# ruanjinchen/Point-Cloud-Flow-Matching

Measured on AMD Instinct MI355X. Metric: train-step points/sec (B=8, N=20000, xyz+rgb) at 1/2/4/8 MI355X; Chamfer ms, higher is better.
Workload: dtype fp32 ContextNet (scatter/gather ops fp32; Conv3d + 1x1 convs as bf16x3 split-operand matrix-core products, fp32 accumulate, ~2^-16 per product vs the reference's default cuDNN TF32 2^-11) + bf16 autocast per-point MLP head (reference AMP config; its per-cloud B-row layers -- embeddings, FiLM affines

## Files before the change

### point-cloud-flow-matching_amd/csrc/pointwise.hip

```cpp
#include <algorithm>
#include <cstdlib>

#include "mfma_x3.hpp"

namespace pcfm {
namespace {

inline int pad_to(int x, int m) { return (x + m - 1) / m * m; }

__device__ __forceinline__ void out_store(float* p, float v) {
#ifndef PCFM_PW_CACHED_STORE
  nt_st(v, p);
#else
  *p = v;
#endif
}
inline int pw_mpad(int m) { return m > 256 ? pad_to(m, 256) : pad_to(m, 128); }

constexpr int kMaxParts = 4;
struct Parts {
  float* p[kMaxParts];
  int off[kMaxParts + 1];
  int n;
  __device__ __forceinline__ float* row(int b, int c, int N) const {
    int i = 0;
#pragma unroll
// ... 117 lines not shown
        const int dm = (e & 3) + 8 * (e >> 2) + 4 * h;
        const int m = mg + dm;
        const int p = p0 + wc * (TN / 2) + j * 32 + r;
        if (m < M && p < N) out_store(yr + (size_t)dm * N + p, acc[i][j][e] + bv[e]);
      }
  }
}

template <int MASK>
__device__ __forceinline__ float swz_xor(float v) {
  return __builtin_bit_cast(
      float, __builtin_amdgcn_ds_swizzle(__builtin_bit_cast(int, v), (MASK << 10) | 0x1f));
}
template <int K, int MASK>
__device__ __forceinline__ void xpose_reduce_stage(float* v, bool upper) {
#pragma unroll
  for (int k = 0; k < K / 2; ++k) {
    const float keep = upper ? v[k + K / 2] : v[k];
    const float send = upper ? v[k] : v[k + K / 2];
    v[k] = keep + swz_xor<MASK>(send);
  }
}

__device__ __forceinline__ void pw256_epilogue(const f32x16 (&acc)[2][2], const Parts& y,
                                               const float* __restrict__ sbias, int b, int nb,
                                               int M, int N, int m0, int p0, int wr, int wc,
                                               int r, int h, float2* __restrict__ stats) {
  const int pw0 = p0 + wc * 64;
#pragma unroll
  for (int i = 0; i < 2; ++i) {
    const int mg = m0 + wr * 64 + i * 32;
    float* __restrict__ yr = y.row(b, min(mg, M - 1), N);
    float bv[16];
#pragma unroll
    for (int e = 0; e < 16; ++e) bv[e] = sbias[mg - m0 + (e & 3) + 8 * (e >> 2) + 4 * h];
#pragma unroll
    for (int j = 0; j < 2; ++j)
#pragma unroll
      for (int e = 0; e < 16; ++e) {
        const int dm = (e & 3) + 8 * (e >> 2) + 4 * h;
        const int m = mg + dm;
        const int p = pw0 + j * 32 + r;
#ifdef PCFM_EXP_PW_NOSTORE
        if (acc[i][j][e] == 1.2345f)
#endif
        if (m < M && p < N) out_store(yr + (size_t)dm * N + p, acc[i][j][e] + bv[e]);
// ... 12 lines not shown
            float, __builtin_amdgcn_readlane(__builtin_bit_cast(int, v0), 32));
        const float sh = h ? s1 : s0;
        sr = r == e ? sh : sr;
        const float d0 = ok0 ? v0 - sh : 0.0f, d1 = ok1 ? v1 - sh : 0.0f;
        v[e] = d0 + d1;
        v[16 + e] = __builtin_fmaf(d1, d1, d0 * d0);
      }
      xpose_reduce_stage<32, 16>(v, r & 16);
      xpose_reduce_stage<16, 8>(v, r & 8);
      xpose_reduce_stage<8, 4>(v, r & 4);
      xpose_reduce_stage<4, 2>(v, r & 2);
      xpose_reduce_stage<2, 1>(v, r & 1);
      const float q = swz_xor<16>(v[0]);
      const int m = mg + (r & 3) + 8 * ((r >> 2) & 3) + 4 * h;
      if (r < 16 && m < M) {
        const float a = v[0], mu_s = a / (float)nv;
        stats[(size_t)m * P + b * ngroups + pw0 / 64] =
            make_float2(sr + mu_s, fmaxf(__builtin_fmaf(-a, mu_s, q), 0.0f));
      }
    }
  }
}

__global__ void __launch_bounds__(512) __attribute__((amdgpu_waves_per_eu(4, 4)))
    pw_gemm256_kernel(const Parts x, const uint16_t* __restrict__ wh,
                      const uint16_t* __restrict__ wl, const float* __restrict__ bias,
                      int bias_bstride, const Parts y, int K, int M, int N, int Kpad,
                      float2* __restrict__ stats = nullptr) {
  constexpr int TM = 256, TN = 128;
  constexpr int A_ELEMS = TM * kLDR, B_ELEMS = TN * kLDR;
  __shared__ __attribute__((aligned(16))) uint16_t lds[2 * A_ELEMS + 2 * B_ELEMS];
  __shared__ float sbias[TM];
  const int b = blockIdx.z, m0 = blockIdx.y * TM, p0 = blockIdx.x * TN;
  const int t = threadIdx.x, lane = t & 63;
  if (t < TM) sbias[t] = bias != nullptr ? bias[b * bias_bstride + min(m0 + t, M - 1)] : 0.0f;
  const int w = __builtin_amdgcn_readfirstlane(t >> 6);
  const int wr = w >> 1, wc = w & 1, r = lane & 31, h = lane >> 5;
  constexpr int CPT = kKT * TN / 512;
  const int sp = t % TN, ch = __builtin_amdgcn_readfirstlane((t / TN) * CPT);
  const int pt = p0 + sp;
  const bool pok = pt < N;
  const int ptc = pok ? pt : N - 1;
  const int arow = t >> 1, ahalf = (t & 1) * 16;
  const int nsteps = Kpad / kKT;

  uint4 ra0 = {}, ra1 = {}, ra2 = {}, ra3 = {};
  float rb[CPT];
  const __amdgpu_buffer_rsrc_t rwh = __builtin_amdgcn_make_buffer_rsrc(
      const_cast<uint16_t*>(wh), (short)0, 0x7FFFFFF0, 0x00020000);
  const __amdgpu_buffer_rsrc_t rwl = __builtin_amdgcn_make_buffer_rsrc(
      const_cast<uint16_t*>(wl), (short)0, 0x7FFFFFF0, 0x00020000);
  const int aoff = ((m0 + arow) * Kpad + ahalf) * 2;
  auto load_a = [&](int s) {
#ifdef PCFM_EXP_PW_NOW
    if (s > 0) return;
#endif
    const int so = s * kKT * 2;
    ra0 = __builtin_bit_cast(uint4, __builtin_amdgcn_raw_buffer_load_b128(rwh, aoff, so, 0));
// ... 70 lines not shown
        }
    }
  };

  load_a(0);
  load_b(0, rb);
  store(0, rb);
  __syncthreads();
  for (int s = 0; s < nsteps; ++s) {
    if (s + 1 < nsteps) {
      load_a(s + 1);
      load_b(s + 1, rb);
    }
    __builtin_amdgcn_sched_barrier(0);
#ifndef PCFM_EXP_PW_NOMFMA
    mfma_step();
#else
    acc[0][0][0] += (float)lds[t];
#endif
    __syncthreads();
    if (s + 1 < nsteps) store(s + 1, rb);
    __syncthreads();
  }
  pw256_epilogue(acc, y, sbias, b, (int)gridDim.z,
                 M, N, m0, p0, wr, wc, r, h, stats);
}

constexpr int kSW = 8;
#ifndef PCFM_PW_STREAM_PF
#define PCFM_PW_STREAM_PF 1
#endif
__device__ __forceinline__ bf16x8 split8(const float (&v)[8], bf16x8& lo) {
  bf16x8 hi;
#pragma unroll
  for (int j = 0; j < 8; ++j) {
    hi[j] = (__bf16)v[j];
    lo[j] = (__bf16)(v[j] - (float)hi[j]);
  }
  return hi;
}

__device__ __forceinline__ const float* uniform_ptr(const float* p) {
  const unsigned long long u = (unsigned long long)p;
  const unsigned lo = __builtin_amdgcn_readfirstlane((unsigned)u);
  const unsigned hi = __builtin_amdgcn_readfirstlane((unsigned)(u >> 32));
  return (const float*)(((unsigned long long)hi << 32) | lo);
}

// ... 463 lines not shown
__global__ void __launch_bounds__(256)
    pw_wgrad_reduce_kernel(const float* __restrict__ part, size_t total, int S,
                           float* __restrict__ dw) {
  __shared__ float red[4][64];
  const int cl = threadIdx.x & 63, grp = threadIdx.x >> 6;
  const size_t i = (size_t)blockIdx.x * 64 + cl;
  float sum = 0.0f;
  if (i < total) {
    int q = grp;
    for (; q + 12 < S; q += 16) {
      float v[4];
#pragma unroll
      for (int u = 0; u < 4; ++u) v[u] = part[(size_t)(q + 4 * u) * total + i];
#pragma unroll
      for (int u = 0; u < 4; ++u) sum = sum + v[u];
    }
    for (; q < S; q += 4) sum = sum + part[(size_t)q * total + i];
  }
  red[grp][cl] = sum;
  __syncthreads();
  if (grp == 0 && i < total) dw[i] = ((red[0][cl] + red[1][cl]) + red[2][cl]) + red[3][cl];
}

bool pw_wgrad_wide(int cin, int cout) {
#ifdef PCFM_PW_NO256
  return false;
#else
  return cin % 256 == 0 && cout % 256 == 0;
#endif
}

int pw_wgrad_splits(int B, int cin, int cout, int N) {
  if (pw_wgrad_wide(cin, cout)) {
    const long long tiles = (long long)(cout / 256) * ((cin + 255) / 256);
    const long long steps = (long long)B * ((N + kKT - 1) / kKT);
    long long s = std::max(1LL, ((long long)kCUs + tiles - 1) / tiles);
    s = std::min(s, std::max(1LL, steps / 16));
    return (int)std::min(s, 256LL);
  }
#ifndef PCFM_PW_WG_BPC
#define PCFM_PW_WG_BPC 2
#endif
#ifndef PCFM_PW_WG_MINSTEPS
#define PCFM_PW_WG_MINSTEPS 8
#endif
#ifndef PCFM_PW_WG_CAP
// ... 38 lines not shown

enum class PwPath { Stream128, Tile256, Tile128, Tile64 };

static PwPath pw_path(int b, int cin, int cout, int n) {
  const int Mpad = pw_mpad(cout), Kpad = pad_to(cin, kKT);
  const long long big = (long long)ceil_div(n, 128) * (Mpad / 128) * b;
#ifndef PCFM_PW_NOSTREAM
  if (Mpad == 128 && Kpad <= 256 && cin % 32 == 0 && cout % 32 == 0) return PwPath::Stream128;
#endif
#ifndef PCFM_PW_NO256
  if (Mpad % 256 == 0 && big / 2 >= 2 * kCUs) return PwPath::Tile256;
#endif
  return big >= 2 * kCUs ? PwPath::Tile128 : PwPath::Tile64;
}

static bool pw_path_has_stats(PwPath p) {
  if (p == PwPath::Stream128) {
    const char* e = std::getenv("PCFM_PW_STREAM_STATS");
    return PCFM_PW_STREAM_PF < 2 && (e == nullptr || e[0] != '0');
  }
  return p == PwPath::Tile256;
}
static int pw_stats_group(PwPath p) { return p == PwPath::Stream128 ? 32 : 64; }

static int pw_gemm_launch(const Parts& x, const void* wsplit, const float* bias, int bias_bstride,
                          int b, int cin, int cout, int n, const Parts& y, hipStream_t st,
                          float2* stats = nullptr) {
  const int Mpad = pw_mpad(cout), Kpad = pad_to(cin, kKT);
  const size_t total = (size_t)Mpad * Kpad;
  const uint16_t* wh = (const uint16_t*)wsplit;
  const PwPath path = pw_path(b, cin, cout, n);
  PCFM_CHECK_ARG(stats == nullptr || pw_path_has_stats(path),
                 "pointwise_gemm: BatchNorm statistics requested for a shape whose kernel has "
                 "no statistics epilogue (b=%d cin=%d cout=%d n=%d)", b, cin, cout, n);
  if (path == PwPath::Stream128) {
    const uint16_t* wl_img = wh + total;
    const long long tiles = (long long)b * ceil_div(n, 32);
    const size_t lds = (size_t)2 * 128 * (Kpad + 8) * sizeof(uint16_t);
    const int per_cu = lds <= 80 * 1024 ? 2 : 1;
    const int slices = Mpad / 128;
    const long long cap = std::max(8LL, ((long long)kCUs * per_cu / slices) & ~7LL);
    const int grid = (int)std::max(1LL, std::min((tiles + kSW - 1) / kSW, cap));
    const void* kfn = nullptr;
    switch (Kpad / 32) {
#define PW_STREAM_CASE(NC)                                                                 \
  case NC:                                                                                 \
    kfn = stats != nullptr ? (const void*)pw_stream128_kernel<NC, true>                    \
                           : (const void*)pw_stream128_kernel<NC, false>;                  \
    break;
      PW_STREAM_CASE(1) PW_STREAM_CASE(2) PW_STREAM_CASE(3) PW_STREAM_CASE(4)
      PW_STREAM_CASE(5) PW_STREAM_CASE(6) PW_STREAM_CASE(7) PW_STREAM_CASE(8)
#undef PW_STREAM_CASE
    }
    const int e = allow_big_lds(kfn);
    if (e) return e;
    void* args[] = {(void*)&x,    (void*)&wh,  (void*)&wl_img, (void*)&bias,
                    (void*)&bias_bstride, (void*)&y, (void*)&cin, (void*)&cout,
                    (void*)&n,    (void*)&b,   (void*)&stats};
    const hipError_t le = hipLaunchKernel(kfn, dim3(grid, slices), dim3(kSW * 64), args, lds, st);
    if (le != hipSuccess) {
      set_error("pointwise_gemm: launch failed");
      return (int)le;
    }
    return check_launch("pointwise_gemm");
  }
  if (path == PwPath::Tile256) {
    const dim3 g256(ceil_div(n, 128), Mpad / 256, b);
    hipLaunchKernelGGL(pw_gemm256_kernel, g256, dim3(512), 0, st, x, wh, wh + total, bias,
                       bias_bstride, y, cin, cout, n, Kpad, stats);
    return check_launch("pointwise_gemm");
  }
  if (path == PwPath::Tile128) {
    hipLaunchKernelGGL((pw_gemm_kernel<128, 128>), dim3(ceil_div(n, 128), Mpad / 128, b),
                       dim3(256), 0, st, x, wh, wh + total, bias, bias_bstride, y, cin, cout, n,
                       Kpad);
  } else {
    hipLaunchKernelGGL((pw_gemm_kernel<64, 64>), dim3(ceil_div(n, 64), Mpad / 64, b), dim3(256),
                       0, st, x, wh, wh + total, bias, bias_bstride, y, cin, cout, n, Kpad);
  }
  return check_launch("pointwise_gemm");
}

static bool make_parts(int np, float* const* ptr, const int* width, int align, Parts& q,
                       int& total) {
  if (np < 1 || np > kMaxParts || ptr == nullptr || width == nullptr) return false;
  q = Parts{};
  q.n = np;
  total = 0;
  for (int i = 0; i < np; ++i) {
    if (width[i] <= 0 || ptr[i] == nullptr) return false;
// ... 11 lines not shown
                                   int cin, int cout, int n, float* y, void* stream) {
  PCFM_CHECK_ARG(pw_ok(b, cin, cout, n), "pointwise_gemm: bad shape b=%d cin=%d cout=%d n=%d", b,
                 cin, cout, n);
  if (b == 0 || n == 0) return PCFM_OK;
  return pw_gemm_launch(one_part(x, cin), wsplit, bias, 0, b, cin, cout, n, one_part(y, cout),
                        (hipStream_t)stream);
}

extern "C" int pcfm_pointwise_bnstats_groups(int b, int cin, int cout, int n) {
  if (!pw_ok(b, cin, cout, n) || b <= 0 || n <= 0) return 0;
  const PwPath p = pw_path(b, cin, cout, n);
  if (!pw_path_has_stats(p)) return 0;
  return b * ceil_div(n, pw_stats_group(p));
}

extern "C" int pcfm_pointwise_gemm_bnstats(const float* x, const void* wsplit, const float* bias,
                                           int b, int cin, int cout, int n, float* y,
                                           float* stats, void* stream) {
  PCFM_CHECK_ARG(pcfm_pointwise_bnstats_groups(b, cin, cout, n) > 0 && stats != nullptr,
                 "pointwise_gemm_bnstats: unsupported shape b=%d cin=%d cout=%d n=%d", b, cin,
                 cout, n);
  return pw_gemm_launch(one_part(x, cin), wsplit, bias, 0, b, cin, cout, n, one_part(y, cout),
                        (hipStream_t)stream, reinterpret_cast<float2*>(stats));
}

extern "C" int pcfm_pointwise_gemm_parts(int nx, const float* const* x, const int* xw,
                                         const void* wsplit, const float* bias, int bias_per_batch,
                                         int b, int n, int ny, float* const* y, const int* yw,
                                         void* stream) {
  Parts px, py;
  int cin = 0, cout = 0;
  PCFM_CHECK_ARG(make_parts(nx, const_cast<float* const*>(x), xw, kKT, px, cin),
                 "pointwise_gemm_parts: bad input parts (1..%d, widths %% %d)", kMaxParts, kKT);
  PCFM_CHECK_ARG(make_parts(ny, y, yw, 128, py, cout),
                 "pointwise_gemm_parts: bad output parts (1..%d, widths %% 128)", kMaxParts);
  PCFM_CHECK_ARG(pw_ok(b, cin, cout, n), "pointwise_gemm_parts: bad shape b=%d cin=%d cout=%d n=%d",
                 b, cin, cout, n);
  if (b == 0 || n == 0) return PCFM_OK;
  return pw_gemm_launch(px, wsplit, bias, bias_per_batch ? cout : 0, b, cin, cout, n, py,
                        (hipStream_t)stream);
}

static int pw_wgrad_launch(const Parts& x, const float* grad_y, int b, int cin, int cout, int n,
                           float* grad_w, void* ws, hipStream_t st) {
  const size_t total = (size_t)cout * cin;
  const int S = pw_wgrad_splits(b, cin, cout, n);
// ... 53 lines not shown
```

### point-cloud-flow-matching_amd/modules/norm_act.py

```python
import torch
import torch.nn.functional as F

__all__ = ["bn_act", "conv_bn_act", "gn_film_residual", "post_gn_film_residual"]

_DEBUG_CHECKS = __import__("os").environ.get("PCFM_DEBUG_CHECKS") == "1"
_BN_FROM_GEMM = __import__("os").environ.get("PCFM_BN_FROM_GEMM", "1") != "0"


class _BNAct(torch.autograd.Function):
    @staticmethod
    def forward(ctx, x, weight, bias, running_mean, running_var, nbt, eps, momentum, slope):
        from pcfm import ops
        y, mean, invstd = ops.bn_act_forward(x, weight, bias, eps, slope, momentum, running_mean,
                                             running_var, nbt)
        ctx.save_for_backward(x, weight, bias, mean, invstd)
        ctx.slope = slope
        return y

    @staticmethod
    def backward(ctx, dy):
        from pcfm import ops
        x, weight, bias, mean, invstd = ctx.saved_tensors
        dx, dgamma, dbeta, _ = ops.bn_act_backward(dy, x, weight, bias, mean, invstd, ctx.slope)
        return dx, dgamma, dbeta, None, None, None, None, None, None


def _fusable(x: torch.Tensor, bn) -> bool:
    if not (x.is_cuda and x.dtype == torch.float32 and x.dim() >= 3 and bn.training
            and bn.affine and bn.track_running_stats and bn.momentum is not None
# ... 8 lines not shown
    if _fusable(x, bn):
        return _BNAct.apply(x.contiguous(), bn.weight, bn.bias, bn.running_mean, bn.running_var,
                            _nbt(bn), float(bn.eps), float(bn.momentum), float(slope))
    y = bn(x)
    return F.relu(y, inplace=True) if slope == 0 else F.leaky_relu(y, slope, inplace=True)


class _PwBnAct(torch.autograd.Function):

    @staticmethod
    def forward(ctx, x, w, b, gamma, beta, rmean, rvar, nbt, eps, momentum, slope):
        from pcfm import ops
        ys = ops.pointwise_forward_bnstats(x, w, b) if _BN_FROM_GEMM else None
        if ys is not None:
            y, stats = ys
            z, mean, invstd = ops.bn_act_forward_parts(y, stats, gamma, beta, eps, slope,
                                                       momentum, rmean, rvar, nbt)
        else:
            y = ops.pointwise_forward(x, w, b)
            z, mean, invstd = ops.bn_act_forward(y, gamma, beta, eps, slope, momentum, rmean,
                                                 rvar, nbt)
        ctx.save_for_backward(x, w, y, gamma, beta, mean, invstd)
        ctx.slope, ctx.has_bias = slope, b is not None
        return z

    @staticmethod
    def backward(ctx, dz):
        from pcfm import ops
        x, w, y, gamma, beta, mean, invstd = ctx.saved_tensors
        dy, dgamma, dbeta, db = ops.bn_act_backward(dz, y, gamma, beta, mean, invstd, ctx.slope,
                                                    want_dbias_in=ctx.has_bias)
        dx = ops.pointwise_backward_data(dy, w) if ctx.needs_input_grad[0] else None
        dw = ops.pointwise_backward_weight(x, dy).view_as(w) if ctx.needs_input_grad[1] else None
        return dx, dw, db, dgamma, dbeta, None, None, None, None, None, None


class _Conv3dBnAct(torch.autograd.Function):

    @staticmethod
    def forward(ctx, x, w, b, gamma, beta, rmean, rvar, nbt, eps, momentum, slope):
        from pcfm import ops
        bsz, cin, r = x.shape[0], x.shape[1], x.shape[2]
        cout = w.shape[0]
        xs = ops.conv3d_split(x)
        y = ops.conv3d_igemm_split(xs, ops.conv3d_prep_weight(w, False), b, bsz, cin, cout, r,
                                   "conv3d_fwd")
        z, mean, invstd = ops.bn_act_forward(y, gamma, beta, eps, slope, momentum, rmean, rvar,
                                             nbt)
        ctx.save_for_backward(xs, w, y, gamma, beta, mean, invstd)
        ctx.slope, ctx.has_bias, ctx.dims = slope, b is not None, (bsz, cin, cout, r)
        return z

    @staticmethod
    def backward(ctx, dz):
        from pcfm import ops
# ... 192 lines not shown
    return x + (y * (1.0 + gamma[:, :, None]) + beta[:, :, None])


_POST_GN_FUSED = __import__("os").environ.get("PCFM_POST_GN_FUSED", "1") != "0"


class _PostGNFiLMRes(torch.autograd.Function):

    @staticmethod
    def forward(ctx, x, w, b, g_bn, bt_bn, rm, rv, nbt, eps, momentum, slope, gn_w, gn_b, gamma,
                beta, groups, gn_eps):
        from pcfm import ops
        ys = ops.pointwise_forward_bnstats(x, w, b) if _BN_FROM_GEMM else None
        if ys is not None:
            y, stats = ys
            mean, invstd = ops.bn_forward_stats(y, eps, momentum, rm, rv, nbt, parts=stats)
        else:
            y = ops.pointwise_forward(x, w, b)
            mean, invstd = ops.bn_forward_stats(y, eps, momentum, rm, rv, nbt)
        out, gm, grs = ops.gn_film_res_forward_bnin(y, mean, invstd, g_bn, bt_bn, slope, gn_w,
                                                    gn_b, gamma, beta, groups, gn_eps)
        ctx.save_for_backward(x, w, y, g_bn, bt_bn, mean, invstd, gn_w, gn_b, gamma, gm, grs)
        ctx.slope, ctx.groups, ctx.has_bias = slope, groups, b is not None
        return out

    @staticmethod
    def backward(ctx, dout):
        from pcfm import ops
        x, w, y, g_bn, bt_bn, mean, invstd, gn_w, gn_b, gamma, gm, grs = ctx.saved_tensors
        dz, dgnw, dgnb, dgamma, dbeta, bnpart = ops.gn_film_res_backward_bnin(
            dout, y, mean, invstd, g_bn, bt_bn, ctx.slope, gn_w, gn_b, gamma, gm, grs, ctx.groups)
        dy, dg_bn, db_bn, db = ops.bn_act_backward_parts(dz, y, g_bn, bt_bn, mean, invstd, bnpart,
                                                         ctx.slope, want_dbias_in=ctx.has_bias)
        del dz
        dx = ops.pointwise_backward_data(dy, w) if ctx.needs_input_grad[0] else None
        dw = ops.pointwise_backward_weight(x, dy).view_as(w) if ctx.needs_input_grad[1] else None
        return (dx, dw, db, dg_bn, db_bn, None, None, None, None, None, None, dgnw, dgnb, dgamma,
                dbeta, None, None)


def post_gn_film_residual(post, norm, x: torch.Tensor, gamma: torch.Tensor, beta: torch.Tensor):
    layers = post.layers
    conv, bn = layers[0], layers[1]
    fused = (_POST_GN_FUSED and len(layers) == 3 and isinstance(layers[2], torch.nn.ReLU)
             and x.is_cuda and x.dtype == torch.float32 and x.dim() == 3
             and _fusable_pre(bn) and hasattr(conv, "x3_ok") and conv.x3_ok(x)
             and conv.bias is not None and isinstance(norm, torch.nn.GroupNorm) and norm.affine
             and x.shape[2] % 4 == 0 and conv.out_channels <= 1024
             and x.shape[0] * conv.out_channels < 65536 and x.shape[0] * x.shape[2] > 1
             and conv.out_channels % norm.num_groups == 0
             and gamma.dtype == torch.float32 and beta.dtype == torch.float32)
    if not fused:
        return gn_film_residual(post(x), norm, gamma, beta)
    return _PostGNFiLMRes.apply(
        x.contiguous(), conv.weight, conv.bias, bn.weight, bn.bias, bn.running_mean,
        bn.running_var, _nbt(bn), float(bn.eps), float(bn.momentum), 0.0, norm.weight, norm.bias,
        gamma, beta, int(norm.num_groups), float(norm.eps))
```

### point-cloud-flow-matching_amd/modules/pvconv.py

```python
import torch
import torch.nn as nn
import torch.nn.functional as TF

import modules.functional as F
from modules.norm_act import (_BN_FROM_GEMM, _fusable_pre, _nbt, _pair_head, _pair_tail,
                              conv_bn_act_pair, pair_fusable)
from modules.se import SE3d
from modules.shared_mlp import SharedMLP
from modules.voxel_conv import VoxelConv3d
from modules.voxelization import Voxelization

__all__ = ["PVConv"]


def _conv_bn_lrelu(cin, cout, kernel_size):
    return [
        VoxelConv3d(cin, cout, kernel_size, stride=1, padding=kernel_size // 2),
        nn.BatchNorm3d(cout, eps=1e-4),
        nn.LeakyReLU(0.1, True),
    ]


_SE_FUSED = __import__("os").environ.get("PCFM_SE_FUSED", "1") != "0"


def _se_scale(m, w1, w2):
    return torch.sigmoid(TF.linear(TF.relu(TF.linear(m, w1)), w2))


# ... 63 lines not shown
        else:
            y_pf, parts = ops.pointwise_forward(f, pw, pb), None
        pm, pis = ops.bn_forward_stats(y_pf, peps, pmom, prm, prv, pnbt, parts=parts)
        xs, y1, m1, is1, z1s, y2 = _pair_head(x, w1, b1, g1, bt1, rm1, rv1, nbt1, w2, b2, eps1,
                                              mom1, slope1, occ)
        mse, m2, is2 = ops.bn_act_forward_rowmean(y2, g2, bt2, eps2, slope2, mom2, rm2, rv2,
                                                  nbt2)
        sw1, sw2 = sw1.contiguous(), sw2.contiguous()
        s, hid = ops.se_mlp_forward(mse, sw1, sw2)
        shared = plans.devox_corners(coords, r)
        out, inds, wgts = ops.trilinear_devoxelize_bn_scale_add(
            r, shared is None, coords, y2, m2, is2, g2, bt2, slope2, s, y_pf,
            add_bn=(pm, pis, pg, pbt, 0.0))
        if shared is not None:
            inds, wgts = shared
        else:
            plans.put_devox_corners(coords, r, inds, wgts)
        ctx.save_for_backward(xs, w1, y1, g1, bt1, m1, is1, z1s, w2, y2, g2, bt2, m2, is2,
                              inds, wgts, mse, s, hid, sw1, sw2, f, pw, y_pf, pg, pbt, pm, pis)
        ctx.points, ctx.r, ctx.occ = coords, r, occ
        ctx.slopes = (slope1, slope2)
        ctx.has_bias = (b1 is not None, b2 is not None, pb is not None)
        ctx.dims = (x.shape[0], x.shape[1], w1.shape[0], w2.shape[0], x.shape[2])
        return out

    @staticmethod
    def backward(ctx, dout):
        from pcfm import ops, plans
        (xs, w1, y1, g1, bt1, m1, is1, z1s, w2, y2, g2, bt2, m2, is2, inds, wgts, mse, s, hid,
         sw1, sw2, f, pw, y_pf, pg, pbt, pm, pis) = ctx.saved_tensors
        dout = dout.contiguous()
        dy_pf, dpg, dpbt, dpb = ops.bn_act_backward(dout, y_pf, pg, pbt, pm, pis, 0.0,
                                                    want_dbias_in=ctx.has_bias[2])
        df = ops.pointwise_backward_data(dy_pf, pw) if ctx.needs_input_grad[18] else None
        dpw = ops.pointwise_backward_weight(f, dy_pf).view_as(pw)
        del dy_pf
        if plans.ENABLED:
            plan = plans.devox_bwd_plan(ctx.points, inds, wgts, ctx.r)
            g = ops.trilinear_devoxelize_backward_planned(dout, plan)
        else:
            g = ops.trilinear_devoxelize_backward(dout, inds, wgts, ctx.r)
        g = g.view(y2.shape)
        rowstats = ops.bn_se_backward_stats(g, y2, m2, is2, g2, bt2, ctx.slopes[1])
        v = y2[0, 0].numel()
        dmv, dsw1, dsw2 = ops.se_mlp_backward(mse, hid, s, rowstats[0], sw1, sw2, 1.0 / v)
        gys2, dg2, dbt2, db2 = ops.bn_se_backward_apply_split(
            g, y2, m2, is2, g2, bt2, s, dmv, rowstats, ctx.slopes[1],
            want_dbias_in=ctx.has_bias[1])
        del g
        dx, dw1, db1, dg1, dbt1, dw2 = _pair_tail(gys2, xs, w1, y1, g1, bt1, m1, is1, z1s, w2,
                                                  ctx.slopes[0], ctx.has_bias[0], ctx.dims,
                                                  ctx.occ, ctx.needs_input_grad[0])
        return (dx, dw1, db1, dg1, dbt1, None, None, None, dw2, db2, dg2, dbt2, None, None, None,
                dsw1, dsw2, None, df, dpw, dpb, dpg, dpbt, None, None, None, None, None, None,
                None, None, None, None, None, None, None)

# ... 94 lines not shown
```

### point-cloud-flow-matching_amd/pcfm/_lib.py

```python
from __future__ import annotations

import ctypes
import os
import threading

_HERE = os.path.dirname(os.path.abspath(__file__))
LIB_PATH = os.path.join(os.path.dirname(_HERE), "csrc", "libpcfm_hip.so")
LIB_PATH = os.environ.get("PCFM_LIB", LIB_PATH)

_P = ctypes.c_void_p
_I = ctypes.c_int
_F = ctypes.c_float
_Z = ctypes.c_size_t
_L = ctypes.c_longlong
_D = ctypes.c_double
_DP = ctypes.POINTER(ctypes.c_double)

SIGNATURES = {
    "pcfm_abi_version": (_I, []),
    "pcfm_last_error": (ctypes.c_char_p, []),
    "pcfm_avg_voxelize_fwd_workspace_bytes": (_Z, [_I, _I, _I, _I]),
    "pcfm_avg_voxelize_fwd": (_I, [_P, _P, _I, _I, _I, _I, _P, _P, _P, _P, _Z, _P]),
    "pcfm_avg_voxelize_bwd": (_I, [_P, _P, _P, _I, _I, _I, _I, _P, _P]),
    "pcfm_trilinear_devoxelize_fwd": (_I, [_P, _P, _I, _I, _I, _I, _I, _P, _P, _P, _P]),
# ... 119 lines not shown
}

ABI_VERSION = 20

ND_SIGNATURES = {
    "pcfm_chamfer_nd_abi_version": (_I, []),
    "pcfm_chamfer_nd_supported": (_I, [_I]),
    "pcfm_chamfer_nd_workspace_bytes": (_Z, [_I, _I, _I, _I]),
    "pcfm_chamfer_nd_fwd": (_I, [_P, _P, _I, _I, _I, _I, _P, _P, _P, _P, _P, _Z, _P]),
    "pcfm_chamfer_nd_bwd": (_I, [_P, _P, _I, _I, _I, _I, _P, _P, _P, _P, _P, _P, _P]),
}

ND_ABI_VERSION = 1

CROSS_SIGNATURES = {
    "pcfm_chamfer_cross_abi_version": (_I, []),
    "pcfm_chamfer_cross_supported": (_I, [_I]),
    "pcfm_chamfer_cross_workspace_bytes": (_Z, [_I, _I, _I, _I, _I]),
    "pcfm_chamfer_cross_fwd": (_I, [_P, _P, _I, _I, _I, _I, _I, _P, _P, _P, _Z, _P]),
}

CROSS_ABI_VERSION = 1

_lock = threading.Lock()
_lib = None


class PcfmError(RuntimeError):
    """A pcfm_* entry point returned a non-zero status."""


def load() -> ctypes.CDLL:
    global _lib
    if _lib is not None:
        return _lib
    with _lock:
        if _lib is None:
            if not os.path.exists(LIB_PATH):
                raise RuntimeError(
                    f"pcfm: HIP library {LIB_PATH} is not built; run "
                    "`python -c 'import __graft_entry__ as g; g.build()'` "
                    "(HIP tensors have no fallback)")
            lib = ctypes.CDLL(LIB_PATH)
            for table in (SIGNATURES, ND_SIGNATURES, CROSS_SIGNATURES):
                for name, (res, args) in table.items():
                    fn = getattr(lib, name)
                    fn.restype = res
                    fn.argtypes = args
            v = lib.pcfm_abi_version()
            if v != ABI_VERSION:
                raise RuntimeError(f"pcfm: ABI version {v} != expected {ABI_VERSION}; rebuild")
            v = lib.pcfm_chamfer_nd_abi_version()
            if v != ND_ABI_VERSION:
                raise RuntimeError(f"pcfm: chamfer_nd ABI version {v} != expected "
                                   f"{ND_ABI_VERSION}; rebuild")
            v = lib.pcfm_chamfer_cross_abi_version()
            if v != CROSS_ABI_VERSION:
                raise RuntimeError(f"pcfm: chamfer_cross ABI version {v} != expected "
                                   f"{CROSS_ABI_VERSION}; rebuild")
            _lib = lib
    return _lib


def call(name: str, *args) -> None:
    lib = load()
    rc = getattr(lib, name)(*args)
    if rc != 0:
        msg = lib.pcfm_last_error().decode(errors="replace")
        raise PcfmError(f"{name} failed (status {rc}): {msg}")


def query(name: str, *args) -> int:
    return int(getattr(load(), name)(*args))
```

### point-cloud-flow-matching_amd/pcfm/ops.py

```python
from __future__ import annotations

import ctypes
import types

import torch

from . import _lib, cpu_ops


def _check_cuda(x: torch.Tensor, name: str) -> None:
    if not (isinstance(x, torch.Tensor) and x.is_cuda):
        raise RuntimeError(f"{name} must be a CUDA tensor")


def _check_contig(x: torch.Tensor, name: str) -> None:
    if not x.is_contiguous():
        raise RuntimeError(f"{name} must be a contiguous tensor")


def _check_float(x: torch.Tensor, name: str) -> None:
    if x.dtype != torch.float32:
        raise RuntimeError(f"{name} must be a float tensor")


# ... 864 lines not shown
        return None
    img = pointwise_prep_weight(weight, False)
    y = torch.empty((b, cout, n), dtype=torch.float32, device=x.device)
    stats = torch.empty((cout, groups, 2), dtype=torch.float32, device=x.device)
    bias_c = bias.contiguous() if bias is not None else None
    bias_p = _ptr(bias_c) if bias_c is not None else None
    with _timed("pointwise_fwd", 2 * b * n * cin * cout, x, "mfma"):
        _lib.call("pcfm_pointwise_gemm_bnstats", _ptr(x), _ptr(img), bias_p, b, cin, cout, n,
                  _ptr(y), _ptr(stats), _stream(x))
    return y, stats


def pointwise_backward_data(grad_y: torch.Tensor, weight: torch.Tensor) -> torch.Tensor:
    _check(grad_y, "grad_output", "f")
    g = grad_y.contiguous()
    b, cout, n = g.shape
    cin = weight.shape[1]
    img = pointwise_prep_weight(weight, True)
    dx = torch.empty((b, cin, n), dtype=torch.float32, device=g.device)
    with _timed("pointwise_bwd_data", 2 * b * n * cin * cout, g, "mfma"):
        _lib.call("pcfm_pointwise_gemm", _ptr(g), _ptr(img), None, b, cout, cin, n, _ptr(dx),
                  _stream(g))
    return dx


def pointwise_backward_weight(x: torch.Tensor, grad_y: torch.Tensor) -> torch.Tensor:
    _check(x, "input", "f")
    _check(grad_y, "grad_output", "f")
    x, g = x.contiguous(), grad_y.contiguous()
    b, cin, n = x.shape
    cout = g.shape[1]
    ws = _workspace(_lib.query("pcfm_pointwise_wgrad_workspace_bytes", b, cin, cout, n), x)
    dw = torch.empty((cout, cin), dtype=torch.float32, device=x.device)
    with _timed("pointwise_wgrad", 2 * b * n * cin * cout, x, "mfma"):
        _lib.call("pcfm_pointwise_wgrad", _ptr(x), _ptr(g), b, cin, cout, n, _ptr(dw), _ptr(ws),
                  ws.numel(), _stream(x))
    return dw


def _parts(ts):
    ptrs = (ctypes.c_void_p * len(ts))(*[_ptr(t) for t in ts])
    widths = (ctypes.c_int * len(ts))(*[int(t.shape[1]) for t in ts])
    return ptrs, widths


def pointwise_forward_parts(xs, weight: torch.Tensor, bias, bias_per_batch: bool = False):
# ... 558 lines not shown
```

Measured before the change: 5.809 million.

## Fuse BatchNorm-backward channel sums into pointwise backward-data GEMM epilogue

Adds a variant of the 256-wide pointwise GEMM whose epilogue, when computing dx for a layer fed by a BN+LeakyReLU, reloads the pre-activation z and produces per-channel partial sums of the masked gradient and gradient*xhat. A small fold kernel reduces these partials, and a handover cache passes them to the upstream BN backward so it can skip its own reduction pass over dy and z. This replaces a full-tensor reduction read with extra epilogue work and z reads inside the GEMM, plus Python-side identity-cache bookkeeping. It only applies on the Tile256 path for supported shapes.

```diff
diff --git a/include/pcfm_bn_parts.h b/include/pcfm_bn_parts.h
--- /dev/null
+++ b/include/pcfm_bn_parts.h
@@ -0,0 +1,27 @@
+#ifndef PCFM_BN_PARTS_H
+#define PCFM_BN_PARTS_H
+
+#include <stddef.h>
+
+#ifdef __cplusplus
+extern "C" {
+#endif
+
+#define PCFM_BN_PARTS_ABI_VERSION 1
+
+int pcfm_bn_parts_abi_version(void);
+
+int pcfm_pointwise_bnbwd_groups(int b, int cin, int cout, int n);
+
+int pcfm_pointwise_gemm_bnbwd(const float* x, const void* wsplit, int b, int cin, int cout, int n,
+                              float* y, const float* z, const float* mean, const float* invstd,
+                              const float* gamma, const float* beta, float slope, float* part,
+                              void* stream);
+
+int pcfm_bn_parts_fold(const float* part, int c, int P, float* folded, void* stream);
+
+#ifdef __cplusplus
+}
+#endif
+
+#endif
diff --git a/point-cloud-flow-matching_amd/csrc/pointwise.hip b/point-cloud-flow-matching_amd/csrc/pointwise.hip
--- a/point-cloud-flow-matching_amd/csrc/pointwise.hip
+++ b/point-cloud-flow-matching_amd/csrc/pointwise.hip
@@ -2,6 +2,7 @@
 #include <cstdlib>
 
 #include "mfma_x3.hpp"
+#include "../../include/pcfm_bn_parts.h"
 
 namespace pcfm {
 namespace {
@@ -165,6 +166,33 @@
   }
 }
 
+struct BnBwdEpi {
+  const float* z;
+  const float* mean;
+  const float* invstd;
+  const float* gamma;
+  const float* beta;
+  float slope;
+  float2* part;
+};
+
+__device__ __forceinline__ void bnbwd_stage(const BnBwdEpi& bw, int m0, int M, int rows, int t,
+                                            float4* __restrict__ sc) {
+  if (t < rows) {
+    const int m = min(m0 + t, M - 1);
+    sc[t] = make_float4(bw.mean[m], bw.invstd[m], bw.gamma[m], bw.beta[m]);
+  }
+}
+
+__device__ __forceinline__ void bnbwd_term(float dz, float z, const float4 c, float slope, bool ok,
+                                           float& sg, float& sgx) {
+  const float xh = (z - c.x) * c.y;
+  float g = __builtin_fmaf(xh, c.z, c.w) > 0.0f ? dz : dz * slope;
+  g = ok ? g : 0.0f;
+  sg += g;
+  sgx += g * xh;
+}
+
 __device__ __forceinline__ void pw256_epilogue(const f32x16 (&acc)[2][2], const Parts& y,
                                                const float* __restrict__ sbias, int b, int nb,
                                                int M, int N, int m0, int p0, int wr, int wc,
@@ -223,18 +251,87 @@
   }
 }
 
-__global__ void __launch_bounds__(512) __attribute__((amdgpu_waves_per_eu(4, 4)))
-    pw_gemm256_kernel(const Parts x, const uint16_t* __restrict__ wh,
-                      const uint16_t* __restrict__ wl, const float* __restrict__ bias,
-                      int bias_bstride, const Parts y, int K, int M, int N, int Kpad,
-                      float2* __restrict__ stats = nullptr) {
+__device__ __forceinline__ void pw256_epilogue_bnbwd(const f32x16 (&acc)[2][2], const Parts& y,
+                                                     int b, int nb, int M, int N, int m0, int p0,
+                                                     int wr, int wc, int r, int h,
+                                                     const BnBwdEpi& bw,
+                                                     const float4* __restrict__ sbn) {
+  const int pw0 = p0 + wc * 64;
+  const int mw = m0 + wr * 64;
+  const bool on0 = pw0 < N && mw < M, on1 = pw0 < N && mw + 32 < M;
+  auto zload = [&](int i, float (&zv)[32]) {
+    const __amdgpu_buffer_rsrc_t rs = __builtin_amdgcn_make_buffer_rsrc(
+        const_cast<float*>(bw.z + ((size_t)b * M + mw + 32 * i) * N), (short)0, 0x7FFFFFF0,
+        0x00020000);
+#pragma unroll
+    for (int j = 0; j < 2; ++j) {
+      const int voff = (4 * h * N + min(pw0 + j * 32 + r, N - 1)) * 4;
+#pragma unroll
+      for (int e = 0; e < 16; ++e)
+        zv[16 * j + e] = __builtin_bit_cast(
+            float,
+            __builtin_amdgcn_raw_buffer_load_b32(rs, voff, ((e & 3) + 8 * (e >> 2)) * N * 4, 0));
+    }
+  };
+  auto sums = [&](int i, const float (&zv)[32]) {
+    const int mg = mw + 32 * i;
+    const int ngroups = (N + 63) / 64, P = nb * ngroups;
+    const bool ok0 = pw0 + r < N, ok1 = pw0 + 32 + r < N;
+    float v[16];
+#pragma unroll
+    for (int e = 0; e < 16; ++e) {
+      const float4 c = sbn[mg - m0 + (e & 3) + 8 * (e >> 2) + 4 * h];
+      float sg = 0.0f, sgx = 0.0f;
+      bnbwd_term(acc[i][0][e] + 0.0f, zv[e], c, bw.slope, ok0, sg, sgx);
+      bnbwd_term(acc[i][1][e] + 0.0f, zv[16 + e], c, bw.slope, ok1, sg, sgx);
+      v[e] = ((r & 16) ? sgx : sg) + swz_xor<16>((r & 16) ? sg : sgx);
+    }
+    xpose_reduce_stage<16, 8>(v, r & 8);
+    xpose_reduce_stage<8, 4>(v, r & 4);
+    xpose_reduce_stage<4, 2>(v, r & 2);
+    xpose_reduce_stage<2, 1>(v, r & 1);
+    const float q = swz_xor<16>(v[0]);
+    const int m = mg + (r & 3) + 8 * ((r >> 2) & 3) + 4 * h;
+    if (r < 16 && m < M) bw.part[(size_t)m * P + b * ngroups + pw0 / 64] = make_float2(v[0], q);
+  };
+  auto stores = [&](int i) {
+    const int mg = mw + 32 * i;
+    float* __restrict__ yr = y.row(b, min(mg, M - 1), N);
+#pragma unroll
+    for (int j = 0; j < 2; ++j)
+#pragma unroll
+      for (int e = 0; e < 16; ++e) {
+        const int dm = (e & 3) + 8 * (e >> 2) + 4 * h;
+        const int p = pw0 + j * 32 + r;
+        if (mg + dm < M && p < N) out_store(yr + (size_t)dm * N + p, acc[i][j][e] + 0.0f);
+      }
+  };
+  float za[32], zb[32];
+  if (on0) {
+    zload(0, za);
+    sums(0, za);
+  }
+  if (on1) zload(1, zb);
+  stores(0);
+  if (on1) sums(1, zb);
+  stores(1);
+}
+
+template <bool BW>
+__device__ __forceinline__ void pw_gemm256_body(const Parts& x, const uint16_t* __restrict__ wh,
+                                                const uint16_t* __restrict__ wl,
+                                                const float* __restrict__ bias, int bias_bstride,
+                                                const Parts& y, int K, int M, int N, int Kpad,
+                                                float2* __restrict__ stats, const BnBwdEpi& bw) {
   constexpr int TM = 256, TN = 128;
   constexpr int A_ELEMS = TM * kLDR, B_ELEMS = TN * kLDR;
   __shared__ __attribute__((aligned(16))) uint16_t lds[2 * A_ELEMS + 2 * B_ELEMS];
   __shared__ float sbias[TM];
+  __shared__ float4 sbn[BW ? TM : 1];
   const int b = blockIdx.z, m0 = blockIdx.y * TM, p0 = blockIdx.x * TN;
   const int t = threadIdx.x, lane = t & 63;
   if (t < TM) sbias[t] = bias != nullptr ? bias[b * bias_bstride + min(m0 + t, M - 1)] : 0.0f;
+  if (BW) bnbwd_stage(bw, m0, M, TM, t, sbn);
   const int w = __builtin_amdgcn_readfirstlane(t >> 6);
   const int wr = w >> 1, wc = w & 1, r = lane & 31, h = lane >> 5;
   constexpr int CPT = kKT * TN / 512;
@@ -351,8 +448,28 @@
     if (s + 1 < nsteps) store(s + 1, rb);
     __syncthreads();
   }
-  pw256_epilogue(acc, y, sbias, b, (int)gridDim.z,
-                 M, N, m0, p0, wr, wc, r, h, stats);
+  if (BW) {
+    pw256_epilogue_bnbwd(acc, y, b, (int)gridDim.z, M, N, m0, p0, wr, wc, r, h, bw, sbn);
+  } else {
+    pw256_epilogue(acc, y, sbias, b, (int)gridDim.z,
+                   M, N, m0, p0, wr, wc, r, h, stats);
+  }
+}
+
+__global__ void __launch_bounds__(512) __attribute__((amdgpu_waves_per_eu(4, 4)))
+    pw_gemm256_kernel(const Parts x, const uint16_t* __restrict__ wh,
+                      const uint16_t* __restrict__ wl, const float* __restrict__ bias,
+                      int bias_bstride, const Parts y, int K, int M, int N, int Kpad,
+                      float2* __restrict__ stats = nullptr) {
+  pw_gemm256_body<false>(x, wh, wl, bias, bias_bstride, y, K, M, N, Kpad, stats, BnBwdEpi{});
+}
+
+__global__ void __launch_bounds__(512) __attribute__((amdgpu_waves_per_eu(4, 4)))
+    pw_gemm256_bnbwd_kernel(const Parts x, const uint16_t* __restrict__ wh,
+                            const uint16_t* __restrict__ wl, const float* __restrict__ bias,
+                            int bias_bstride, const Parts y, int K, int M, int N, int Kpad,
+                            const BnBwdEpi bw) {
+  pw_gemm256_body<true>(x, wh, wl, bias, bias_bstride, y, K, M, N, Kpad, nullptr, bw);
 }
 
 constexpr int kSW = 8;
@@ -862,6 +979,42 @@
   if (grp == 0 && i < total) dw[i] = ((red[0][cl] + red[1][cl]) + red[2][cl]) + red[3][cl];
 }
 
+__global__ void __launch_bounds__(256)
+    bn_parts_fold_kernel(const float2* __restrict__ part, int P, float2* __restrict__ folded) {
+  __shared__ float sh[8];
+  const int c = blockIdx.x, t = threadIdx.x;
+  const float2* __restrict__ pc = part + (size_t)c * P;
+  float a = 0.0f, q = 0.0f;
+  int p = t;
+  for (; p + 3 * 256 < P; p += 4 * 256) {
+    float2 v[4];
+#pragma unroll
+    for (int u = 0; u < 4; ++u) v[u] = pc[p + u * 256];
+#pragma unroll
+    for (int u = 0; u < 4; ++u) {
+      a += v[u].x;
+      q += v[u].y;
+    }
+  }
+  for (; p < P; p += 256) {
+    const float2 v = pc[p];
+    a += v.x;
+    q += v.y;
+  }
+#pragma unroll
+  for (int off = 32; off > 0; off >>= 1) {
+    a += __shfl_xor(a, off, 64);
+    q += __shfl_xor(q, off, 64);
+  }
+  if ((t & 63) == 0) {
+    sh[2 * (t >> 6)] = a;
+    sh[2 * (t >> 6) + 1] = q;
+  }
+  __syncthreads();
+  if (t == 0)
+    folded[c] = make_float2(((sh[0] + sh[2]) + sh[4]) + sh[6], ((sh[1] + sh[3]) + sh[5]) + sh[7]);
+}
+
 bool pw_wgrad_wide(int cin, int cout) {
 #ifdef PCFM_PW_NO256
   return false;
@@ -946,10 +1099,14 @@
   return p == PwPath::Tile256;
 }
 static int pw_stats_group(PwPath p) { return p == PwPath::Stream128 ? 32 : 64; }
+static bool pw_path_has_bnbwd(PwPath p, int cout, int n) {
+  if (cout % 32 != 0 || (long long)n * 128 >= (1LL << 31)) return false;
+  return p == PwPath::Tile256;
+}
 
 static int pw_gemm_launch(const Parts& x, const void* wsplit, const float* bias, int bias_bstride,
                           int b, int cin, int cout, int n, const Parts& y, hipStream_t st,
-                          float2* stats = nullptr) {
+                          float2* stats = nullptr, const BnBwdEpi* bnbwd = nullptr) {
   const int Mpad = pw_mpad(cout), Kpad = pad_to(cin, kKT);
   const size_t total = (size_t)Mpad * Kpad;
   const uint16_t* wh = (const uint16_t*)wsplit;
@@ -957,6 +1114,10 @@
   PCFM_CHECK_ARG(stats == nullptr || pw_path_has_stats(path),
                  "pointwise_gemm: BatchNorm statistics requested for a shape whose kernel has "
                  "no statistics epilogue (b=%d cin=%d cout=%d n=%d)", b, cin, cout, n);
+  PCFM_CHECK_ARG(bnbwd == nullptr ||
+                     (stats == nullptr && bias == nullptr && pw_path_has_bnbwd(path, cout, n)),
+                 "pointwise_gemm: BatchNorm backward sums requested for a shape whose kernel "
+                 "has no such epilogue (b=%d cin=%d cout=%d n=%d)", b, cin, cout, n);
   if (path == PwPath::Stream128) {
     const uint16_t* wl_img = wh + total;
     const long long tiles = (long long)b * ceil_div(n, 32);
@@ -990,6 +1151,11 @@
   }
   if (path == PwPath::Tile256) {
     const dim3 g256(ceil_div(n, 128), Mpad / 256, b);
+    if (bnbwd != nullptr) {
+      hipLaunchKernelGGL(pw_gemm256_bnbwd_kernel, g256, dim3(512), 0, st, x, wh, wh + total, bias,
+                         bias_bstride, y, cin, cout, n, Kpad, *bnbwd);
+      return check_launch("pointwise_gemm");
+    }
     hipLaunchKernelGGL(pw_gemm256_kernel, g256, dim3(512), 0, st, x, wh, wh + total, bias,
                        bias_bstride, y, cin, cout, n, Kpad, stats);
     return check_launch("pointwise_gemm");
@@ -1047,6 +1213,39 @@
                  cout, n);
   return pw_gemm_launch(one_part(x, cin), wsplit, bias, 0, b, cin, cout, n, one_part(y, cout),
                         (hipStream_t)stream, reinterpret_cast<float2*>(stats));
+}
+
+extern "C" int pcfm_bn_parts_abi_version(void) { return PCFM_BN_PARTS_ABI_VERSION; }
+
+extern "C" int pcfm_pointwise_bnbwd_groups(int b, int cin, int cout, int n) {
+  if (!pw_ok(b, cin, cout, n) || b <= 0 || n <= 0) return 0;
+  const PwPath p = pw_path(b, cin, cout, n);
+  if (!pw_path_has_bnbwd(p, cout, n)) return 0;
+  return b * ceil_div(n, pw_stats_group(p));
+}
+
+extern "C" int pcfm_pointwise_gemm_bnbwd(const float* x, const void* wsplit, int b, int cin,
+                                         int cout, int n, float* y, const float* z,
+                                         const float* mean, const float* invstd,
+                                         const float* gamma, const float* beta, float slope,
+                                         float* part, void* stream) {
+  PCFM_CHECK_ARG(pcfm_pointwise_bnbwd_groups(b, cin, cout, n) > 0,
+                 "pointwise_gemm_bnbwd: unsupported shape b=%d cin=%d cout=%d n=%d", b, cin, cout,
+                 n);
+  PCFM_CHECK_ARG(z != nullptr && mean != nullptr && invstd != nullptr && gamma != nullptr &&
+                     beta != nullptr && part != nullptr,
+                 "pointwise_gemm_bnbwd: BatchNorm operands missing");
+  const BnBwdEpi bw{z, mean, invstd, gamma, beta, slope, reinterpret_cast<float2*>(part)};
+  return pw_gemm_launch(one_part(x, cin), wsplit, nullptr, 0, b, cin, cout, n, one_part(y, cout),
+                        (hipStream_t)stream, nullptr, &bw);
+}
+
+extern "C" int pcfm_bn_parts_fold(const float* part, int c, int P, float* folded, void* stream) {
+  PCFM_CHECK_ARG(c > 0 && P > 0 && part != nullptr && folded != nullptr,
+                 "bn_parts_fold: bad arguments c=%d P=%d", c, P);
+  hipLaunchKernelGGL(bn_parts_fold_kernel, dim3(c), dim3(256), 0, (hipStream_t)stream,
+                     reinterpret_cast<const float2*>(part), P, reinterpret_cast<float2*>(folded));
+  return check_launch("bn_parts_fold");
 }
 
 extern "C" int pcfm_pointwise_gemm_parts(int nx, const float* const* x, const int* xw,
diff --git a/point-cloud-flow-matching_amd/modules/norm_act.py b/point-cloud-flow-matching_amd/modules/norm_act.py
--- a/point-cloud-flow-matching_amd/modules/norm_act.py
+++ b/point-cloud-flow-matching_amd/modules/norm_act.py
@@ -5,6 +5,46 @@
 
 _DEBUG_CHECKS = __import__("os").environ.get("PCFM_DEBUG_CHECKS") == "1"
 _BN_FROM_GEMM = __import__("os").environ.get("PCFM_BN_FROM_GEMM", "1") != "0"
+_BN_BWD_FROM_GEMM = __import__("os").environ.get("PCFM_BN_BWD_FROM_GEMM", "1") != "0"
+
+
+class _BnBwdHandover:
+
+    def __init__(self):
+        from pcfm.plans import IdentityCache
+        self._c = IdentityCache()
+        self.taken = 0
+
+    def offer(self, out, bn):
+        if _BN_BWD_FROM_GEMM:
+            self._c.put(out, "bn", bn)
+
+    def _pop(self, t, tag):
+        v = self._c.get(t, tag)
+        if v is not None:
+            self._c._d.pop((id(t), tag), None)
+        return v
+
+    def source(self, x):
+        return self._pop(x, "bn") if _BN_BWD_FROM_GEMM else None
+
+    def backward_data(self, bn, dy, w):
+        from pcfm import ops
+        r = ops.pointwise_backward_data_bnparts(dy, w, *bn) if bn is not None else None
+        if r is None:
+            return ops.pointwise_backward_data(dy, w)
+        dx, part = r
+        self._c.put(dx, "part", part)
+        return dx
+
+    def claim(self, dout):
+        part = self._pop(dout, "part") if _BN_BWD_FROM_GEMM else None
+        if part is not None:
+            self.taken += 1
+        return part
+
+
+bn_bwd_handover = _BnBwdHandover()
 
 
 class _BNAct(torch.autograd.Function):
@@ -59,6 +99,7 @@
                                                  rvar, nbt)
         ctx.save_for_backward(x, w, y, gamma, beta, mean, invstd)
         ctx.slope, ctx.has_bias = slope, b is not None
+        ctx.bn_src = bn_bwd_handover.source(x)
         return z
 
     @staticmethod
@@ -67,7 +108,8 @@
         x, w, y, gamma, beta, mean, invstd = ctx.saved_tensors
         dy, dgamma, dbeta, db = ops.bn_act_backward(dz, y, gamma, beta, mean, invstd, ctx.slope,
                                                     want_dbias_in=ctx.has_bias)
-        dx = ops.pointwise_backward_data(dy, w) if ctx.needs_input_grad[0] else None
+        bn_src, ctx.bn_src = ctx.bn_src, None
+        dx = bn_bwd_handover.backward_data(bn_src, dy, w) if ctx.needs_input_grad[0] else None
         dw = ops.pointwise_backward_weight(x, dy).view_as(w) if ctx.needs_input_grad[1] else None
         return dx, dw, db, dgamma, dbeta, None, None, None, None, None, None
 
@@ -306,6 +348,7 @@
                                                     gn_b, gamma, beta, groups, gn_eps)
         ctx.save_for_backward(x, w, y, g_bn, bt_bn, mean, invstd, gn_w, gn_b, gamma, gm, grs)
         ctx.slope, ctx.groups, ctx.has_bias = slope, groups, b is not None
+        ctx.bn_src = bn_bwd_handover.source(x)
         return out
 
     @staticmethod
@@ -317,7 +360,8 @@
         dy, dg_bn, db_bn, db = ops.bn_act_backward_parts(dz, y, g_bn, bt_bn, mean, invstd, bnpart,
                                                          ctx.slope, want_dbias_in=ctx.has_bias)
         del dz
-        dx = ops.pointwise_backward_data(dy, w) if ctx.needs_input_grad[0] else None
+        bn_src, ctx.bn_src = ctx.bn_src, None
+        dx = bn_bwd_handover.backward_data(bn_src, dy, w) if ctx.needs_input_grad[0] else None
         dw = ops.pointwise_backward_weight(x, dy).view_as(w) if ctx.needs_input_grad[1] else None
         return (dx, dw, db, dg_bn, db_bn, None, None, None, None, None, None, dgnw, dgnb, dgamma,
                 dbeta, None, None)
diff --git a/point-cloud-flow-matching_amd/modules/pvconv.py b/point-cloud-flow-matching_amd/modules/pvconv.py
--- a/point-cloud-flow-matching_amd/modules/pvconv.py
+++ b/point-cloud-flow-matching_amd/modules/pvconv.py
@@ -4,7 +4,7 @@
 
 import modules.functional as F
 from modules.norm_act import (_BN_FROM_GEMM, _fusable_pre, _nbt, _pair_head, _pair_tail,
-                              conv_bn_act_pair, pair_fusable)
+                              bn_bwd_handover, conv_bn_act_pair, pair_fusable)
 from modules.se import SE3d
 from modules.shared_mlp import SharedMLP
 from modules.voxel_conv import VoxelConv3d
@@ -114,6 +114,7 @@
         ctx.slopes = (slope1, slope2)
         ctx.has_bias = (b1 is not None, b2 is not None, pb is not None)
         ctx.dims = (x.shape[0], x.shape[1], w1.shape[0], w2.shape[0], x.shape[2])
+        bn_bwd_handover.offer(out, (y_pf, pm, pis, pg, pbt, 0.0))
         return out
 
     @staticmethod
@@ -121,9 +122,14 @@
         from pcfm import ops, plans
         (xs, w1, y1, g1, bt1, m1, is1, z1s, w2, y2, g2, bt2, m2, is2, inds, wgts, mse, s, hid,
          sw1, sw2, f, pw, y_pf, pg, pbt, pm, pis) = ctx.saved_tensors
+        bnpart = bn_bwd_handover.claim(dout)
         dout = dout.contiguous()
-        dy_pf, dpg, dpbt, dpb = ops.bn_act_backward(dout, y_pf, pg, pbt, pm, pis, 0.0,
-                                                    want_dbias_in=ctx.has_bias[2])
+        if bnpart is not None:
+            dy_pf, dpg, dpbt, dpb = ops.bn_act_backward_parts(
+                dout, y_pf, pg, pbt, pm, pis, bnpart, 0.0, want_dbias_in=ctx.has_bias[2])
+        else:
+            dy_pf, dpg, dpbt, dpb = ops.bn_act_backward(dout, y_pf, pg, pbt, pm, pis, 0.0,
+                                                        want_dbias_in=ctx.has_bias[2])
         df = ops.pointwise_backward_data(dy_pf, pw) if ctx.needs_input_grad[18] else None
         dpw = ops.pointwise_backward_weight(f, dy_pf).view_as(pw)
         del dy_pf
diff --git a/point-cloud-flow-matching_amd/pcfm/_lib.py b/point-cloud-flow-matching_amd/pcfm/_lib.py
--- a/point-cloud-flow-matching_amd/pcfm/_lib.py
+++ b/point-cloud-flow-matching_amd/pcfm/_lib.py
@@ -165,6 +165,16 @@
 
 CROSS_ABI_VERSION = 1
 
+BN_PARTS_SIGNATURES = {
+    "pcfm_bn_parts_abi_version": (_I, []),
+    "pcfm_pointwise_bnbwd_groups": (_I, [_I, _I, _I, _I]),
+    "pcfm_pointwise_gemm_bnbwd": (_I, [_P, _P, _I, _I, _I, _I, _P, _P, _P, _P, _P, _P, _F, _P,
+                                       _P]),
+    "pcfm_bn_parts_fold": (_I, [_P, _I, _I, _P, _P]),
+}
+
+BN_PARTS_ABI_VERSION = 1
+
 _lock = threading.Lock()
 _lib = None
 
@@ -185,7 +195,7 @@
                     "`python -c 'import __graft_entry__ as g; g.build()'` "
                     "(HIP tensors have no fallback)")
             lib = ctypes.CDLL(LIB_PATH)
-            for table in (SIGNATURES, ND_SIGNATURES, CROSS_SIGNATURES):
+            for table in (SIGNATURES, ND_SIGNATURES, CROSS_SIGNATURES, BN_PARTS_SIGNATURES):
                 for name, (res, args) in table.items():
                     fn = getattr(lib, name)
                     fn.restype = res
@@ -201,6 +211,10 @@
             if v != CROSS_ABI_VERSION:
                 raise RuntimeError(f"pcfm: chamfer_cross ABI version {v} != expected "
                                    f"{CROSS_ABI_VERSION}; rebuild")
+            v = lib.pcfm_bn_parts_abi_version()
+            if v != BN_PARTS_ABI_VERSION:
+                raise RuntimeError(f"pcfm: bn_parts ABI version {v} != expected "
+                                   f"{BN_PARTS_ABI_VERSION}; rebuild")
             _lib = lib
     return _lib
 
diff --git a/point-cloud-flow-matching_amd/pcfm/ops.py b/point-cloud-flow-matching_amd/pcfm/ops.py
--- a/point-cloud-flow-matching_amd/pcfm/ops.py
+++ b/point-cloud-flow-matching_amd/pcfm/ops.py
@@ -910,6 +910,31 @@
         _lib.call("pcfm_pointwise_gemm", _ptr(g), _ptr(img), None, b, cout, cin, n, _ptr(dx),
                   _stream(g))
     return dx
+
+
+def pointwise_backward_data_bnparts(grad_y: torch.Tensor, weight: torch.Tensor, z: torch.Tensor,
+                                    mean, invstd, gamma, beta, slope: float):
+    _check(grad_y, "grad_output", "f")
+    _check(z, "z", "f")
+    g = grad_y.contiguous()
+    b, cout, n = g.shape
+    cin = weight.shape[1]
+    if tuple(z.shape) != (b, cin, n):
+        return None
+    groups = _lib.query("pcfm_pointwise_bnbwd_groups", b, cout, cin, n)
+    if groups <= 0:
+        return None
+    img = pointwise_prep_weight(weight, True)
+    dx = torch.empty((b, cin, n), dtype=torch.float32, device=g.device)
+    raw = torch.empty((cin, groups, 2), dtype=torch.float32, device=g.device)
+    part = torch.empty((cin, 1, 2), dtype=torch.float32, device=g.device)
+    with _timed("pointwise_bwd_data", 2 * b * n * cin * cout, g, "mfma"):
+        _lib.call("pcfm_pointwise_gemm_bnbwd", _ptr(g), _ptr(img), b, cout, cin, n, _ptr(dx),
+                  _ptr(z), _ptr(mean), _ptr(invstd), _ptr(gamma), _ptr(beta), float(slope),
+                  _ptr(raw), _stream(g))
+    with _timed("bn_act_bwd", 4 * raw.numel(), g):
+        _lib.call("pcfm_bn_parts_fold", _ptr(raw), cin, groups, _ptr(part), _stream(g))
+    return dx, part
 
 
 def pointwise_backward_weight(x: torch.Tensor, grad_y: torch.Tensor) -> torch.Tensor:
```

After: 5.820 million, median of 6. About the same (+0.2%).
